# sqliteai/sqlite-vector

Measured on AMD Instinct MI355X. Metric: vectors scanned/sec, L2 top-20 over Nx384 f32, higher is better.
Workload: dtype f32; 1 GPU; 10Mx384 f32 L2 top-20 single-query; rows_per_gpu=10000000, dim=384, k=20, backend=HIP gfx950 x1

## Files before the change

### sqlite-vector_amd/csrc/vg_api.hip

```cpp
#include "vg_internal.h"

#include "vg_scan.h"


typedef void (*scan_fn_t)(ScanArgs);
scan_fn_t vg_pick_scan_kernel_ex(int vtype, int acc, int U);

typedef VgShape Shape;

static const int kAllowedU[] = {1, 2, 3, 4, 6, 8};

static int max_chunks_per_lane(int vtype, int acc, bool bf16_l2_u3) {
    if (vtype == VG_TYPE_F16) return 6;
    if (vtype == VG_TYPE_BF16) return (acc == A_L2 && !bf16_l2_u3) ? 6 : 3;
    return 8;
}

struct ShapeEnv { bool f16_round3, pref_round1, bf16_l2_u3, int_short_round3, force_long; int lpr_log2, u; };
static ShapeEnv shape_env() {
    ShapeEnv e;
    e.f16_round3 = vg_sw(SW_VG_SHAPE_F16_ROUND3, 0) != 0;
    e.pref_round1 = vg_sw(SW_VG_SHAPE_PREF_ROUND1, 0) != 0;
    e.bf16_l2_u3 = vg_sw(SW_VG_SHAPE_BF16_L2_U3, 0) != 0;
    e.int_short_round3 = vg_sw(SW_VG_SHAPE_INT_SHORT_ROUND3, 0) != 0;
// ... 143 lines not shown
        case VG_DIST_COSINE: return A_COS;
        case VG_DIST_DOT: return A_DOT;
        case VG_DIST_L1: return A_L1;
    }
    return -1;
}

static const char *type_tag(int t) {
    switch (t) { case VG_TYPE_F32: return "f32"; case VG_TYPE_F16: return "f16"; case VG_TYPE_BF16: return "bf16";
                 case VG_TYPE_U8: return "u8"; case VG_TYPE_I8: return "i8"; }
    return "?";
}
static const char *acc_tag(int a) {
    switch (a) { case A_L2: return "l2"; case A_COS: return "cos"; case A_DOT: return "dot"; case A_L1: return "l1"; case A_COSN: return "cosn"; }
    return "?";
}


extern "C" const char *vg_scan_kernel_name(vg_corpus *c, int metric) {
    if (!c) return "";
    Shape s;
    int acc = vg_metric_to_acc(metric);
    if (acc < 0 || !choose_shape(c->nch, c->vtype, acc, &s)) return "";
    if (acc == A_COS && (c->vtype == VG_TYPE_F16 || c->vtype == VG_TYPE_BF16) && !s.long_rows && vg_sw(SW_VG_HALF_COSN, 1)) acc = A_COSN;
    if (!s.long_rows && vg_scan_filter_name(c, metric, c->kernel_name, sizeof(c->kernel_name))) return c->kernel_name;
    snprintf(c->kernel_name, sizeof(c->kernel_name), "scan%s_%s_%s_u%d_lpr%d%s", s.long_rows ? "_long" : "",
             type_tag(c->vtype), acc_tag(acc), s.U, 1 << s.lpr_log2, use_nt_loads(c, c->n_rows) ? "_nt" : "");
    return c->kernel_name;
}



#define VG_MERGE_THREADS 1024
__global__ __launch_bounds__(VG_MERGE_THREADS) void vg_merge_kernel(const uint64_t *cand, int nlists, int k,
                                                                    uint64_t *out_keys, const unsigned long long *mirror_src,
                                                                    unsigned long long *mirror_dst) {
    __shared__ __attribute__((aligned(16))) uint8_t scratch[VG_SEL_SCRATCH_BYTES];
    if (mirror_dst && blockIdx.x == 0 && threadIdx.x < 3) mirror_dst[threadIdx.x] = mirror_src[threadIdx.x];
    vg_select_lists(cand + (long long)blockIdx.x * nlists * VG_WAVE, nlists, k, out_keys + (long long)blockIdx.x * VG_WAVE, scratch);
}

int vg_launch_merge(const uint64_t *dev_cand, int nlists, int k, uint64_t *dev_out_keys, int nq, hipStream_t stream) {
    hipLaunchKernelGGL(vg_merge_kernel, dim3((unsigned)nq), dim3(VG_MERGE_THREADS), 0, stream, dev_cand, nlists, k, dev_out_keys,
                       (const unsigned long long *)nullptr, (unsigned long long *)nullptr);
    return (int)hipGetLastError();
}

static int launch_scan(vg_corpus *c, int metric, const uint8_t *dev_query, int k, uint64_t *dev_out_keys,
                       float *dev_out_dist, hipStream_t stream, const ScanPlan &plan = ScanPlan());

int vg_launch_plain_scan(vg_corpus *c, int metric, const uint8_t *dev_query, int k, uint64_t *dev_out_keys, hipStream_t stream,
                         const ScanPlan &plan) {
    return launch_scan(c, metric, dev_query, k, dev_out_keys, nullptr, stream, plan);
}
int vg_launch_merge_one(const uint64_t *dev_cand, int nlists, int k, uint64_t *dev_out_keys, hipStream_t stream,
                        const unsigned long long *mirror_src, unsigned long long *mirror_dst) {
    hipLaunchKernelGGL(vg_merge_kernel, dim3(1), dim3(VG_MERGE_THREADS), 0, stream, dev_cand, nlists, k, dev_out_keys, mirror_src, mirror_dst);
    return (int)hipGetLastError();
}
int vg_plain_scan_shape(const vg_corpus *c, int metric, VgShape *out) {
    choose_shape(c->nch, c->vtype, vg_metric_to_acc(metric), out);
    return 0;
}
long long vg_plain_scan_blocks(const vg_corpus *c, int64_t n_rows, const VgShape &s) {
    const int rpb = VG_WAVE >> s.lpr_log2;
    const long long nbatch = (n_rows + rpb - 1) / rpb;
    const int bpc = std::max(1, std::min(8, vg_sw(SW_VG_BLOCKS_PER_CU, 1)));
    long long blocks = (nbatch + VG_WAVES_PER_BLOCK - 1) / VG_WAVES_PER_BLOCK;
    blocks = std::max<long long>(1, std::min<long long>(blocks, (long long)c->cu_count * bpc));
    blocks = std::min<long long>(blocks, VG_SEL_MAX_HEADS);
    blocks = std::min<long long>(blocks, std::max<long long>(32, nbatch / (2 * VG_WAVES_PER_BLOCK)));
    return blocks;
}

static int launch_scan(vg_corpus *c, int metric, const uint8_t *dev_query, int k, uint64_t *dev_out_keys,
                       float *dev_out_dist, hipStream_t stream, const ScanPlan &plan) {
    int acc = vg_metric_to_acc(metric);
    if (acc < 0) return vg_fail(VG_ERR_INVALID, "unknown distance metric %d", metric);
    const int64_t n_rows = (plan.n_rows >= 0) ? std::min<int64_t>(plan.n_rows, c->n_rows) : c->n_rows;
    if (plan.ref_emit) c->ref_prefix_rows = -1;
    Shape s;
    choose_shape(c->nch, c->vtype, acc, &s);
    const bool whole_prefix = plan.ref_emit && !dev_out_dist && plan.n_rows < 0 && k > 0 && k <= VG_MAX_FUSED_K && !s.long_rows &&
                              n_rows < VG_REF_EMIT_MIN_ROWS;
    if (!whole_prefix && plan.allow_filter && plan.n_rows < 0 && !dev_out_dist && k <= VG_MAX_FUSED_K) {
        int rcf = vg_launch_scan_filter(c, metric, dev_query, k, dev_out_keys, stream, plan.ref_emit, plan.final_out);
        if (rcf != -1) return rcf;
    }
    if (acc == A_COS && (c->vtype == VG_TYPE_F16 || c->vtype == VG_TYPE_BF16) && !s.long_rows && vg_sw(SW_VG_HALF_COSN, 1)) {
        int rcn = vg_ensure_row_norms(c);
        if (rcn != VG_OK) return rcn;
        acc = A_COSN;
        if (stream != c->stream) {
            if (!c->norm_ev) HIP_TRY(hipEventCreateWithFlags(&c->norm_ev, hipEventDisableTiming));
            HIP_TRY(hipEventRecord(c->norm_ev, c->stream));
            HIP_TRY(hipStreamWaitEvent(stream, c->norm_ev, 0));
        }
    }
    const bool emitting = plan.ref_emit && !dev_out_dist && !s.long_rows && plan.n_rows < 0 && k <= VG_MAX_FUSED_K &&
                          n_rows >= VG_REF_EMIT_MIN_ROWS;
    float *store_prefix = plan.store_prefix;
    unsigned long long *emit_reset = plan.emit_reset;
    if (whole_prefix) {
        int rcb = vg_ensure_ref_buffers(c, n_rows);
        if (rcb != VG_OK) return rcb;
        store_prefix = c->d_ref_prefix;
        emit_reset = c->d_below;
        c->ref_prefix_rows = n_rows;
    }
    const bool prefix_pass = store_prefix && !dev_out_dist && !s.long_rows && k > 0;
    scan_fn_t fn = (emitting || prefix_pass) ? vg_pick_scan_kernel_ex(c->vtype, acc, s.U) : pick_kernel(c->vtype, acc, s, use_nt_loads(c, n_rows));
    if (!fn) return vg_fail(VG_ERR_UNSUPPORTED, "no scan kernel for type %s", type_tag(c->vtype));

    const long long blocks = vg_plain_scan_blocks(c, n_rows, s);

    ScanArgs a{};
    a.rows = c->d_rows;
    a.query = dev_query;
    a.cand = plan.lists_out ? plan.lists_out : c->d_cand;
    a.out_dist = dev_out_dist;
    a.n_rows = n_rows;
    a.stride = c->stride;
    a.nch = c->nch;
    a.lpr_log2 = s.lpr_log2;
    a.k = k;
    a.root = (metric == VG_DIST_L2) ? 1 : 0;
    a.dim = c->dim;
    a.row_nn = (acc == A_COSN) ? c->d_xnorm : nullptr;
    a.init_keys = nullptr;
    a.emit = nullptr;
    a.emit_cap = 0;
    a.emit_reset = emit_reset;
    a.order = scan_order_for(c, n_rows);
    if (prefix_pass) a.out_dist = store_prefix;
    else a.emit_reset = nullptr;
    size_t qbytes = (size_t)c->nch * 16;
    if (s.long_rows) {
        const size_t slice = (size_t)VG_WAVE * VG_LONG_U;
        qbytes = ((c->nch + slice - 1) / slice) * slice * 16;
    }
    size_t smem = std::max<size_t>(qbytes, (size_t)VG_PUBLISH_LDS_BYTES);
    a.store_lds_off = 0;
    if (dev_out_dist && !s.long_rows) {
        a.store_lds_off = (int)((qbytes + 255) / 256 * 256);
        smem = std::max<size_t>(smem, (size_t)a.store_lds_off + (size_t)VG_WAVES_PER_BLOCK * VG_STORE_FLOATS * sizeof(float));
    }

    if (c->append_pending && stream != c->stream) HIP_TRY(hipStreamWaitEvent(stream, c->append_ev, 0));

    hipEvent_t *evs = plan.record ? vg_prof_slot(c, (uint8_t)((dev_out_dist == nullptr ? VG_EVF_MERGE : 0) | (emitting ? VG_EVF_PREPASS : 0))) : nullptr;
    if (evs) hipEventRecord(evs[0], stream);
    if (emitting) {
        const int64_t P = vg_ref_prefix_for(n_rows);
        int rcb = vg_ensure_ref_buffers(c, P);
        if (rcb != VG_OK) return rcb;
        ScanPlan pre;
        pre.n_rows = P;
        pre.allow_filter = false;
        pre.record = false;
        pre.store_prefix = c->d_ref_prefix;
        pre.emit_reset = c->d_below;
        int rcp = launch_scan(c, metric, dev_query, k, dev_out_keys, nullptr, stream, pre);
        if (rcp != VG_OK) return rcp;
        a.init_keys = dev_out_keys;
        a.emit = c->d_below;
        a.emit_cap = VG_BELOW_CAP;
        c->ref_prefix_rows = P;
        if (evs) hipEventRecord(evs[1], stream);
    }
    if (smem > 64 * 1024)
        HIP_TRY(hipFuncSetAttribute(reinterpret_cast<const void *>(fn), hipFuncAttributeMaxDynamicSharedMemorySize, (int)smem));
    hipLaunchKernelGGL(fn, dim3((unsigned)blocks), dim3(VG_BLOCK), smem, stream, a);
    if (evs) hipEventRecord(evs[2], stream);
    if (plan.lists_out) {
        if (plan.n_lists_out) *plan.n_lists_out = (int)blocks;
    } else if (!dev_out_dist) {
        hipLaunchKernelGGL(vg_merge_kernel, dim3(1), dim3(VG_MERGE_THREADS), 0, stream,
                           (const uint64_t *)c->d_cand, (int)blocks, k, plan.final_out ? plan.final_out : dev_out_keys,
                           (const unsigned long long *)nullptr, (unsigned long long *)nullptr);
    }
    if (evs) hipEventRecord(evs[3], stream);
    HIP_TRY(hipGetLastError());
    return VG_OK;
}

static bool host_direct(const vg_corpus *c) {
    const int v = vg_sw(SW_VG_HOST_DIRECT, -1);
    if (v >= 0) return v != 0;
    return c->n_rows * c->stride <= (64ll << 20);
}

static void stage_query(vg_corpus *c, const void *query) {
    memset(c->h_query, 0, (size_t)c->stride);
    memcpy(c->h_query, query, (size_t)c->dim * c->es);
}

static void slot_times(vg_corpus *c, int slot, float *scan_ms, float *merge_ms, float *prepass_ms) {
    hipEvent_t *evs = &c->ev[(size_t)slot * VG_PROF_EVS];
    const uint8_t fl = c->ev_flags[(size_t)slot];
    hipEventSynchronize(evs[3]);
    *scan_ms = 0.f; *merge_ms = 0.f; *prepass_ms = 0.f;
    if (fl & VG_EVF_PREPASS) hipEventElapsedTime(prepass_ms, evs[0], evs[1]);
    hipEventElapsedTime(scan_ms, evs[(fl & VG_EVF_PREPASS) ? 1 : 0], evs[2]);
    if (fl & VG_EVF_MERGE) hipEventElapsedTime(merge_ms, evs[2], evs[3]);
}

void vg_collect_timing(vg_corpus *c) {
    if (!c->profiling || c->prof_launches == 0) return;
    slot_times(c, (int)((c->prof_launches - 1) % VG_PROF_RING), &c->last_scan_ms, &c->last_merge_ms, &c->last_prepass_ms);
}

extern "C" float vg_key_distance(uint64_t key) { return vg_sortable_f32((uint32_t)(key >> 32)); }
extern "C" uint32_t vg_key_position(uint64_t key) { return (uint32_t)(key & 0xFFFFFFFFull); }

extern "C" int vg_scan_topk_device(vg_corpus *c, int metric, const void *dev_query, int k, uint64_t *dev_out_keys,
                                   void *stream) {
    if (!c || !dev_query || !dev_out_keys) return vg_fail(VG_ERR_INVALID, "vg_scan_topk_device: NULL argument");
    if (k < 1 || k > VG_MAX_FUSED_K) return vg_fail(VG_ERR_UNSUPPORTED, "vg_scan_topk_device: k must be in 1..%d", VG_MAX_FUSED_K);
    HIP_TRY(hipSetDevice(c->device));
    hipStream_t st = stream ? (hipStream_t)stream : c->stream;
    if (c->n_rows == 0) {
        HIP_TRY(hipMemsetAsync(dev_out_keys, 0xFF, VG_WAVE * sizeof(uint64_t), st));
        return VG_OK;
    }
    return launch_scan(c, metric, (const uint8_t *)dev_query, k, dev_out_keys, nullptr, st);
}

extern "C" int vg_scan_distances_device(vg_corpus *c, int metric, const void *dev_query, float *dev_out_dist, void *stream) {
    if (!c || !dev_query || !dev_out_dist) return vg_fail(VG_ERR_INVALID, "vg_scan_distances_device: NULL argument");
    HIP_TRY(hipSetDevice(c->device));
    if (c->n_rows == 0) return VG_OK;
    return launch_scan(c, metric, (const uint8_t *)dev_query, 0, nullptr, dev_out_dist, stream ? (hipStream_t)stream : c->stream);
}
// ... 279 lines not shown
```

### sqlite-vector_amd/csrc/vg_corpus.hip

```cpp
#include "vg_internal.h"

#include <atomic>
#include <mutex>
#include <utility>
#include <vector>

#include "vg_device.h"


static thread_local std::string g_err;

int vg_fail(int code, const char *fmt, ...) {
    char buf[1024];
    va_list ap;
    va_start(ap, fmt);
    vsnprintf(buf, sizeof(buf), fmt, ap);
    va_end(ap);
    g_err = buf;
    return code;
}

extern "C" const char *vg_last_error(void) { return g_err.c_str(); }
extern "C" void vg_set_last_error_(const char *msg) { g_err = msg ? msg : ""; }

// ... 16 lines not shown
        char arch[64];
        snprintf(arch, sizeof(arch), "%s", p.gcnArchName);
        char *colon = strchr(arch, ':');
        if (colon) *colon = 0;
        snprintf(name, sizeof(name), "HIP %s x%d", arch, n);
    } else {
        snprintf(name, sizeof(name), "HIP");
    }
    return name;
}


struct VgSwitchName { const char *name; int lab; };
static const VgSwitchName vg_switch_names[VGSW_COUNT] = {
    {"VECTORGPU_SHARD_GATHER", 0},
    {"VECTORGPU_SHARD_THREADS", 0},
    {"VG_BATCH_BPC", 1},
    {"VG_BATCH_H_SPLIT", 0},
    {"VG_BATCH_H_WAVES", 0},
    {"VG_BATCH_LONG", 0},
    {"VG_BATCH_LONG_BPC", 1},
    {"VG_BATCH_MFMA", 0},
    {"VG_BATCH_MIN_QUERIES", 1},
    {"VG_BATCH_PREPASS", 1},
    {"VG_BATCH_Q8", 0},
    {"VG_BATCH_SLICE", 0},
    {"VG_BATCH_STAGES", 0},
    {"VG_BATCH_TILE_MAJOR", 0},
    {"VG_BLOCKS_PER_CU", 1},
    {"VG_F32_FILTER", 0},
    {"VG_FILTER_LPR_LOG2", 1},
    {"VG_FILTER_U", 1},
    {"VG_FORCE_LONG", 0},
    {"VG_HALF_COSN", 1},
    {"VG_HOST_DIRECT", 1},
    {"VG_KEYS_DIRECT", 1},
    {"VG_LPR_LOG2", 1},
    {"VG_MULTI_SCAN", 0},
    {"VG_NT", 1},
    {"VG_Q8_TWO_READS", 1},
    {"VG_RADIX_SELECT", 0},
    {"VG_REF_ALWAYS_EMIT", 1},
    {"VG_REF_STORE_MODE", 0},
    {"VG_SCAN_FILTER", 0},
    {"VG_SCAN_FILTER_MIN_MB", 0},
    {"VG_SCAN_FILTER_MIRROR_COPY", 1},
    {"VG_SCAN_FILTER_N4", 0},
    {"VG_SCAN_FILTER_NO_GUARD", 0},
    {"VG_SCAN_FILTER_PREMERGE", 1},
    {"VG_SCAN_FILTER_PREPASS", 1},
    {"VG_SCAN_FILTER_PREPASS_DIV", 1},
    {"VG_SCAN_FILTER_SHADOW", 0},
    {"VG_SCAN_ORDER", 1},
    {"VG_SHAPE_BF16_L2_U3", 1},
    {"VG_SHAPE_F16_ROUND3", 1},
    {"VG_SHAPE_INT_SHORT_ROUND3", 1},
    {"VG_SHAPE_PREF_ROUND1", 1},
    {"VG_U", 1},
};
std::atomic<int> vg_switch_values[VGSW_COUNT];
void vg_switches_read(void) {
    for (int i = 0; i < VGSW_COUNT; ++i) {
        int v = VGSW_UNSET;
#ifndef VG_LAB
        if (!vg_switch_names[i].lab)
#endif
// ... 9 lines not shown
    }
}
__attribute__((constructor)) static void vg_switches_at_load(void) { vg_switches_read(); }
extern "C" void vg_reload_switches(void) { vg_switches_read(); }

extern "C" int vg_corpus_create(int device, int vtype, int dim, int64_t capacity_rows_hint, vg_corpus **out) {
    if (!out) return vg_fail(VG_ERR_INVALID, "vg_corpus_create: out is NULL");
    *out = nullptr;
    vg_switches_read();
    int es = vg_elem_size(vtype);
    if (es == 0) return vg_fail(VG_ERR_INVALID, "vg_corpus_create: unknown vector type %d", vtype);
    if (dim <= 0) return vg_fail(VG_ERR_INVALID, "vg_corpus_create: dimension must be positive (got %d)", dim);
    int ndev = vg_device_count();
    if (ndev <= 0) return vg_fail(VG_ERR_NO_DEVICE, "no HIP device available (the scan path is GPU-only)");
    if (device < 0 || device >= ndev) return vg_fail(VG_ERR_INVALID, "device %d out of range (0..%d)", device, ndev - 1);
    int64_t row_bytes = (int64_t)dim * es;
    if (row_bytes > 128 * 1024) return vg_fail(VG_ERR_UNSUPPORTED, "rows larger than 128 KiB are not supported (dim=%d): the query must fit the CU's 160 KiB LDS", dim);
    HIP_TRY(hipSetDevice(device));
    vg_corpus *c = new vg_corpus();
    c->device = device;
    c->vtype = vtype;
    c->dim = dim;
    c->es = es;
    c->nch = (int)((row_bytes + 15) / 16);
    c->stride = (int64_t)c->nch * 16;
    hipDeviceProp_t p;
    if (hipGetDeviceProperties(&p, device) != hipSuccess) { delete c; return vg_fail(VG_ERR_HIP, "hipGetDeviceProperties failed"); }
    c->cu_count = p.multiProcessorCount;
    c->max_blocks = c->cu_count * 8;
    hipError_t e;
    if ((e = hipStreamCreateWithFlags(&c->stream, hipStreamNonBlocking)) != hipSuccess ||
        (e = hipMalloc(&c->d_query, (size_t)c->stride)) != hipSuccess ||
        (e = hipHostMalloc(&c->h_query, (size_t)c->stride)) != hipSuccess ||
        (e = hipMalloc(&c->d_cand, (size_t)c->max_blocks * VG_WAVE * sizeof(uint64_t))) != hipSuccess ||
        (e = hipMalloc(&c->d_keys, VG_WAVE * sizeof(uint64_t))) != hipSuccess ||
        (e = hipHostMalloc(&c->h_keys, VG_WAVE * sizeof(uint64_t))) != hipSuccess) {
        vg_corpus_destroy(c);
        return vg_fail(VG_ERR_HIP, "vg_corpus_create: device setup failed: %s", hipGetErrorString(e));
    }
    if (capacity_rows_hint > 0) {
        e = hipMalloc(&c->d_rows, (size_t)(capacity_rows_hint * c->stride));
        if (e != hipSuccess) {
            vg_corpus_destroy(c);
            return vg_fail(VG_ERR_NOMEM, "vg_corpus_create: cannot allocate %lld bytes of HBM: %s",
                           (long long)(capacity_rows_hint * c->stride), hipGetErrorString(e));
        }
        c->cap_rows = capacity_rows_hint;
    }
    *out = c;
    return VG_OK;
}

extern "C" void vg_corpus_destroy(vg_corpus *c) {
    if (!c) return;
    hipSetDevice(c->device);
    if (c->stream) hipStreamSynchronize(c->stream);
    if (c->d_rows) hipFree(c->d_rows);
    if (c->d_query) hipFree(c->d_query);
    if (c->h_query) hipHostFree(c->h_query);
    if (c->d_cand) hipFree(c->d_cand);
    if (c->d_cand_pre) hipFree(c->d_cand_pre);
    if (c->d_keys) hipFree(c->d_keys);
    if (c->h_keys) hipHostFree(c->h_keys);
    if (c->d_dist) hipFree(c->d_dist);
    if (c->d_sel_keys) hipFree(c->d_sel_keys);
    if (c->d_sel_sorted) hipFree(c->d_sel_sorted);
    if (c->d_sel_temp) hipFree(c->d_sel_temp);
    for (int i = 0; i < 2; ++i) { if (c->pin[i]) hipHostFree(c->pin[i]); if (c->pin_ev[i]) hipEventDestroy(c->pin_ev[i]); }
    if (c->append_ev) hipEventDestroy(c->append_ev);
    if (c->d_stage) hipFree(c->d_stage);
    if (c->d_bq) hipFree(c->d_bq);
    if (c->h_bq) hipHostFree(c->h_bq);
// ... 677 lines not shown
```

### sqlite-vector_amd/csrc/vg_device.h

```cpp
#pragma once

#include <hip/hip_runtime.h>
#include <stdint.h>

#define VG_EMPTY_KEY 0xFFFFFFFFFFFFFFFFull
#define VG_WAVE 64
#define VG_BLOCK 1024
#define VG_WAVES_PER_BLOCK (VG_BLOCK / VG_WAVE)
#define VG_MAX_FUSED_K 64

enum { T_F32 = 1, T_F16 = 2, T_BF16 = 3, T_U8 = 4, T_I8 = 5 };
enum { M_L2 = 1, M_SQL2 = 2, M_COS = 3, M_DOT = 4, M_L1 = 5 };
enum { A_L2 = 0, A_COS = 1, A_DOT = 2, A_L1 = 3, A_COSN = 4  };

struct ScanArgs {
    const uint8_t *rows;
    const uint8_t *query;
    uint64_t *cand;
    float *out_dist;
    long long n_rows;
    long long stride;
    int nch;
    int lpr_log2;
    int k;
    int root;
    int dim;
    const float *row_nn;
    int store_lds_off;
    const uint64_t *init_keys;
    unsigned long long *emit;
    unsigned emit_cap;
    unsigned long long *emit_reset;
    int order;
    float within_r;
    unsigned long long within_cap;
    const uint64_t *mask;
};


__host__ __device__ inline uint32_t vg_f32_sortable(float d) {
    uint32_t b;
#if defined(__HIP_DEVICE_COMPILE__)
    b = __float_as_uint(d);
#else
    __builtin_memcpy(&b, &d, 4);
#endif
    return b ^ ((b >> 31) ? 0xFFFFFFFFu : 0x80000000u);
}
__host__ __device__ inline float vg_sortable_f32(uint32_t s) {
    uint32_t b = s ^ ((s >> 31) ? 0x80000000u : 0xFFFFFFFFu);
#if defined(__HIP_DEVICE_COMPILE__)
    return __uint_as_float(b);
#else
    float f; __builtin_memcpy(&f, &b, 4); return f;
#endif
}
__host__ __device__ inline uint64_t vg_make_key(float d, uint32_t pos) {
    return ((uint64_t)vg_f32_sortable(d) << 32) | (uint64_t)pos;
}


__device__ inline uint64_t vg_readlane64(uint64_t v, int lane_uniform) {
    uint32_t lo = (uint32_t)__builtin_amdgcn_readlane((int)(uint32_t)v, lane_uniform);
    uint32_t hi = (uint32_t)__builtin_amdgcn_readlane((int)(uint32_t)(v >> 32), lane_uniform);
    return ((uint64_t)hi << 32) | lo;
}

__device__ inline uint64_t vg_wave_shr1(uint64_t v) {
    const uint32_t lo = (uint32_t)__builtin_amdgcn_update_dpp(0, (int)(uint32_t)v, 0x138, 0xf, 0xf, false);
// ... 112 lines not shown
```

### sqlite-vector_amd/csrc/vg_internal.h

```cpp
#pragma once

#include "../../include/vectorgpu.h"
#include "../../include/vectorgpu_diag.h"

#include <hip/hip_runtime.h>

#include <algorithm>
#include <cmath>
#include <cstdarg>
#include <cstdio>
#include <cstdlib>
#include <cstring>
#include <string>
#include <vector>

#define VG_PROF_RING 1024
#define VG_PROF_EVS 4
#define VG_EVF_MERGE 1
#define VG_EVF_PREPASS 2
#define VG_WAVE_HOST 64

int vg_fail(int code, const char *fmt, ...);

#define HIP_TRY(expr)                                                                                     \
    do {                                                                                                  \
        hipError_t e__ = (expr);                                                                          \
        if (e__ != hipSuccess)                                                                            \
            return vg_fail(e__ == hipErrorOutOfMemory ? VG_ERR_NOMEM : VG_ERR_HIP, "%s failed: %s (%s:%d)", \
                           #expr, hipGetErrorString(e__), __FILE__, __LINE__);                            \
    } while (0)


static inline int vg_elem_size(int vtype) {
    switch (vtype) {
        case VG_TYPE_F32: return 4;
        case VG_TYPE_F16: case VG_TYPE_BF16: return 2;
        case VG_TYPE_U8: case VG_TYPE_I8: return 1;
    }
    return 0;
}

struct vg_corpus {
    int device = 0;
    int vtype = 0;
    int dim = 0;
    int es = 0;
    int nch = 0;
    int64_t stride = 0;
    int64_t n_rows = 0;
    int64_t cap_rows = 0;
    uint8_t *d_rows = nullptr;
    std::vector<int64_t> rowids;
    bool rowids_ascending = true;
    int64_t rowid_base = 1;

    hipStream_t stream = nullptr;
    uint8_t *d_query = nullptr;
    uint8_t *h_query = nullptr;
    uint64_t *d_cand = nullptr;
    uint64_t *d_cand_pre = nullptr;
    uint64_t *d_keys = nullptr;
    uint64_t *h_keys = nullptr;
    float *d_dist = nullptr;
    int64_t d_dist_cap = 0;
    int64_t dist_valid_rows = 0;
    unsigned long long *d_below = nullptr;
    uint8_t *h_ref = nullptr;
    size_t h_ref_bytes = 0;
    std::vector<uint64_t> ref_pairs;
    int tie_order = 0;
    float *d_ref_prefix = nullptr;
    int64_t ref_prefix_cap = 0;
    int64_t ref_prefix_rows = -1;
    int ref_hot = 0;
    unsigned long long ref_stats[4] = {0, 0, 0, 0};
    uint64_t *d_sel_keys = nullptr, *d_sel_sorted = nullptr;
    void *d_sel_temp = nullptr;
    uint32_t *d_sel_state = nullptr;
    size_t sel_temp_bytes = 0;
    int64_t sel_cap = 0;
    uint8_t *pin[2] = {nullptr, nullptr};
    hipEvent_t pin_ev[2] = {nullptr, nullptr};
    bool pin_busy[2] = {false, false};
    int pin_idx = 0;
    uint8_t *d_stage = nullptr;
    hipEvent_t append_ev = nullptr;
    bool append_pending = false;
    bool enqueued = false;
    float *d_xnorm = nullptr;
    int64_t xnorm_rows = 0, xnorm_cap = 0;
    hipEvent_t norm_ev = nullptr;
    uint32_t *d_sx = nullptr;
// ... 96 lines not shown
    if (p > VG_REF_PREFIX_MAX) p = VG_REF_PREFIX_MAX;
    return p;
}
int vg_ensure_ref_buffers(vg_corpus *c, int64_t prefix_rows);
#define VG_REF_FIRST_PAIRS 8191
int vg_ref_emitted_enqueue(vg_corpus *c);
int vg_ref_emitted_wait(vg_corpus *c, const float **prefix, int64_t *prefix_rows, unsigned long long **pairs, unsigned long long *count,
                        bool *overflow);
struct VgRefSlots;
void vg_ref_offer_run(VgRefSlots &slots, const float *d, int64_t n, int64_t g0);
int vg_ref_replay_slab(vg_corpus *c, int metric, const void *query, int k, VgRefSlots &slots, int64_t gbase, bool fresh);

static inline void vg_drop_mask(vg_corpus *c) { c->mask_count = -1; c->mask_host.clear(); }
int vg_mask_upload(vg_corpus *c);

static inline hipEvent_t *vg_prof_slot(vg_corpus *c, uint8_t flags) {
    if (!c->profiling) return nullptr;
    const int slot = (int)(c->prof_launches % VG_PROF_RING);
    c->ev_flags[(size_t)slot] = flags;
    ++c->prof_launches;
    return &c->ev[(size_t)slot * VG_PROF_EVS];
}

int vg_metric_to_acc(int metric);
void vg_collect_timing(vg_corpus *c);
int vg_ensure_row_norms(vg_corpus *c);
struct VgShape { int lpr_log2; int U; bool long_rows; };
bool vg_choose_shape(int nch, int vtype, int acc, VgShape *out, int u_cap);
int vg_launch_merge(const uint64_t *dev_cand, int nlists, int k, uint64_t *dev_out_keys, int nq, hipStream_t stream);
int vg_launch_plain_scan(vg_corpus *c, int metric, const uint8_t *dev_query, int k, uint64_t *dev_out_keys, hipStream_t stream,
                         const ScanPlan &plan);
int vg_launch_merge_one(const uint64_t *dev_cand, int nlists, int k, uint64_t *dev_out_keys, hipStream_t stream,
                        const unsigned long long *mirror_src = nullptr, unsigned long long *mirror_dst = nullptr);
int vg_plain_scan_shape(const vg_corpus *c, int metric, VgShape *out);
long long vg_plain_scan_blocks(const vg_corpus *c, int64_t n_rows, const VgShape &s);
int vg_launch_scan_filter(vg_corpus *c, int metric, const uint8_t *dev_query, int k, uint64_t *dev_out_keys, hipStream_t stream,
                          bool ref_emit = false, uint64_t *final_out = nullptr);
int vg_scan_topk_enqueue_plan(vg_corpus *c, int metric, const void *query, int k, bool ref_emit);
bool vg_scan_filter_would_serve(const vg_corpus *c, int metric, int k);
bool vg_scan_filter_policy(const vg_corpus *c);
int vg_ensure_filter_counters(vg_corpus *c);
bool vg_scan_filter_name(vg_corpus *c, int metric, char *out, size_t out_len);
bool vg_batch_keys_are_scan_exact(const vg_corpus *c, int metric, int k);
long long vg_bf16_shadow_stride(const vg_corpus *c);
int vg_ensure_bf16_shadow(vg_corpus *c);
int vg_ensure_q8_shadow(vg_corpus *c);
int vg_multi_queries_per_pass(const vg_corpus *c, int metric);
int vg_launch_scan_multi(vg_corpus *c, int metric, const uint8_t *dev_queries, int k, uint64_t *dev_cand,
                         uint64_t *dev_out_keys, hipStream_t stream);
int vg_multi_plan(const vg_corpus *c, int metric, VgShape *s);
```

### sqlite-vector_amd/csrc/vg_scan.h

```cpp
#pragma once

#include "vg_accum.h"
#include "vg_lists.h"

#define VG_PUBLISH_LDS_BYTES (VG_WAVES_PER_BLOCK * VG_WAVE * 8 + VG_SEL_SCRATCH_BYTES)

__device__ inline void vg_block_publish(uint8_t *smem, uint64_t mine, int k, uint64_t *dst) {
    const int lane = threadIdx.x & (VG_WAVE - 1);
    const int wave = threadIdx.x >> 6;
    uint64_t *lists = reinterpret_cast<uint64_t *>(smem);
    lists[wave * VG_WAVE + lane] = (lane < k) ? mine : VG_EMPTY_KEY;
    __syncthreads();
    vg_select_lists(lists, VG_WAVES_PER_BLOCK, k, dst, smem + VG_WAVES_PER_BLOCK * VG_WAVE * 8);
}

typedef uint32_t vg_u32x4 __attribute__((ext_vector_type(4)));

template <bool NT>
__device__ inline uint4 vg_load16(const uint8_t *p) {
    if (NT) {
        vg_u32x4 v = __builtin_nontemporal_load(reinterpret_cast<const vg_u32x4 *>(p));
        return make_uint4(v.x, v.y, v.z, v.w);
    }
    return *reinterpret_cast<const uint4 *>(p);
}

#ifndef VG_LOAD_PREDICATED
#define VG_LOAD_PREDICATED 0
#endif
static __device__ __attribute__((aligned(16))) uint32_t vg_zero_chunk[4] = {0u, 0u, 0u, 0u};

template <int U, bool NT>
__device__ inline void vg_load_batch(uint4 (&dst)[U], const uint8_t *rows, long long row, long long n_rows,
                                     long long stride, int sub, int lpr, int nch) {
    const uint8_t *p = rows + row * stride + (long long)sub * 16;
#pragma unroll
    for (int u = 0; u < U; ++u) {
        const int c = sub + u * lpr;
        if (VG_LOAD_PREDICATED) {
            uint4 v = make_uint4(0u, 0u, 0u, 0u);
            if (row < n_rows && c < nch) v = vg_load16<NT>(p + (long long)u * lpr * 16);
            dst[u] = v;
        } else {
            const uint8_t *src = (row < n_rows && c < nch) ? p + (long long)u * lpr * 16 : reinterpret_cast<const uint8_t *>(vg_zero_chunk);
            dst[u] = vg_load16<NT>(src);
        }
// ... 27 lines not shown
    queued += __popcll(m);
    if (queued > VG_WITHIN_QUEUE - VG_WAVE) vg_within_flush(queue, queued, out, cap, lane);
}

__device__ inline uint64_t vg_mask_bits(const uint64_t *mask, long long row0, int n, bool in_range) {
    const uint32_t r = (uint32_t)__builtin_amdgcn_readfirstlane((int)(in_range ? (uint32_t)row0 : 0xFFFFFFFFu));
    const bool ok = r != 0xFFFFFFFFu;
    const uint64_t bits = mask[ok ? (r >> 6) : 0u] >> (r & 63u);
    const uint64_t keep = (n >= VG_WAVE) ? ~0ull : ((1ull << (n & 63)) - 1ull);
    return ok ? (bits & keep) : 0ull;
}

template <int VT, int ACC, int U, bool NT, bool EX = false, bool WITHIN = false, bool MASKED = false>
__global__ __launch_bounds__(VG_BLOCK) void vg_scan_kernel(ScanArgs a) {
    extern __shared__ __attribute__((aligned(16))) uint8_t smem[];
    __shared__ VgListExtras ex;
    const int lane = threadIdx.x & (VG_WAVE - 1);
    const int wave = threadIdx.x >> 6;
    const int lpr_log2 = a.lpr_log2;
    const int lpr = 1 << lpr_log2;
    const int rpb = VG_WAVE >> lpr_log2;
    const int sub = lane & (lpr - 1);
    const int rib = lane >> lpr_log2;

    uint4 *qs = reinterpret_cast<uint4 *>(smem);
    for (int c = threadIdx.x; c < a.nch; c += VG_BLOCK) qs[c] = reinterpret_cast<const uint4 *>(a.query)[c];
    const int k = a.k;
    uint64_t mine = VG_EMPTY_KEY;
    uint64_t thr = VG_EMPTY_KEY;
    if constexpr (EX) {
        if (k > 0) thr = vg_list_extras_init(&ex, a.init_keys, k, a.emit, a.emit_cap);
        if (a.emit_reset && blockIdx.x == 0 && threadIdx.x == 0) *a.emit_reset = 0ull;
    }
    __syncthreads();
    uint4 q[U];
#pragma unroll
    for (int u = 0; u < U; ++u) {
        const int c = sub + u * lpr;
        q[u] = (c < a.nch) ? qs[c] : make_uint4(0u, 0u, 0u, 0u);
    }
    const typename Accum<VT, ACC>::QStat qstat = Accum<VT, ACC>::template query_stat<U>(q, lpr_log2);
    const bool store_mode = (WITHIN || MASKED) ? false : EX ? ((a.out_dist != nullptr) && k == 0) : (a.out_dist != nullptr);
    const bool store_too = EX && (a.out_dist != nullptr) && k != 0;

    const long long nbatch = (a.n_rows + rpb - 1) / rpb;
    const long long nwaves = (long long)gridDim.x * VG_WAVES_PER_BLOCK;
    const long long gw = (long long)blockIdx.x * VG_WAVES_PER_BLOCK + wave;
    const int flush_every = VG_STORE_FLOATS / rpb;
    long long per_wave = (nbatch + nwaves - 1) / nwaves;
    per_wave = ((per_wave + flush_every - 1) / flush_every) * flush_every;
    long long wstride = store_mode ? 1 : nwaves;
    long long b = store_mode ? gw * per_wave : gw;
    long long b_end = store_mode ? ((gw + 1) * per_wave < nbatch ? (gw + 1) * per_wave : nbatch) : nbatch;
    if (a.order == 1 && !store_mode) {
        const long long per_block = (nbatch + gridDim.x - 1) / gridDim.x;
        wstride = VG_WAVES_PER_BLOCK;
        b = (long long)blockIdx.x * per_block + wave;
        b_end = ((long long)blockIdx.x + 1) * per_block < nbatch ? ((long long)blockIdx.x + 1) * per_block : nbatch;
    }
    float *line = reinterpret_cast<float *>(smem + a.store_lds_off) + wave * VG_STORE_FLOATS;
    int in_line = 0;
    long long line_row0 = b * rpb;
    uint64_t *wqueue = reinterpret_cast<uint64_t *>(smem + a.store_lds_off) + wave * VG_WITHIN_QUEUE;
    int wqueued = 0;
#ifndef VG_RING_F32
#define VG_RING_F32 0
// ... 94 lines not shown
#pragma unroll
        for (int j = 0; j < NB - 1; ++j) load(buf[j], nn[j], b + j * wstride);
        while (b < b_end) {
#pragma unroll
            for (int j = 0; j < NB; ++j) {
                const long long bj = b + j * wstride;
                load(buf[(j + NB - 1) % NB], nn[(j + NB - 1) % NB], bj + (NB - 1) * wstride);
                if (bj < b_end) process(buf[j], nn[j], bj);
            }
            b += NB * wstride;
        }
    } else {
        load(buf[0], nn[0], b);
        while (b < b_end) {
            const long long bn = b + wstride;
            load(buf[1], nn[1], bn);
            process(buf[0], nn[0], b);
#pragma unroll
            for (int u = 0; u < U; ++u) buf[0][u] = buf[1][u];
            nn[0] = nn[1];
            b = bn;
        }
    }
    if constexpr (WITHIN) {
        if (wqueued > 0) vg_within_flush(wqueue, wqueued, a.emit, a.within_cap, lane);
        return;
    }
    if (store_mode) {
        for (int j = lane; j < in_line * rpb && line_row0 + j < a.n_rows; j += VG_WAVE) a.out_dist[line_row0 + j] = line[j];
        return;
    }

    __syncthreads();
    vg_block_publish(smem, mine, k, a.cand + (long long)blockIdx.x * VG_WAVE);
}

#define VG_LONG_U 2
template <int VT, int ACC, bool NT, bool WITHIN = false, bool MASKED = false>
__global__ __launch_bounds__(VG_BLOCK) void vg_scan_long_kernel(ScanArgs a) {
    extern __shared__ __attribute__((aligned(16))) uint8_t smem[];
    const int lane = threadIdx.x & (VG_WAVE - 1);
    const int wave = threadIdx.x >> 6;
    constexpr int U = VG_LONG_U;
    const int slice = VG_WAVE * U;
    const int S = (a.nch + slice - 1) / slice;
    const int nch_pad = S * slice;

    uint4 *qs = reinterpret_cast<uint4 *>(smem);
    for (int c = threadIdx.x; c < nch_pad; c += VG_BLOCK)
        qs[c] = (c < a.nch) ? reinterpret_cast<const uint4 *>(a.query)[c] : make_uint4(0u, 0u, 0u, 0u);
    __syncthreads();

    typename Accum<VT, ACC>::QStat qstat;
    {
        uint4 q0[U];
#pragma unroll
        for (int u = 0; u < U; ++u) q0[u] = qs[u * VG_WAVE + lane];
        qstat = Accum<VT, ACC>::template query_stat<U>(q0, 6);
        for (int s = 1; s < S; ++s) {
#pragma unroll
            for (int u = 0; u < U; ++u) q0[u] = qs[s * slice + u * VG_WAVE + lane];
            Accum<VT, ACC>::merge_qstat(qstat, Accum<VT, ACC>::template query_stat<U>(q0, 6));
        }
    }

    uint64_t mine = VG_EMPTY_KEY, thr = VG_EMPTY_KEY;
    const int k = a.k;
    const bool store_mode = (WITHIN || MASKED) ? false : (a.out_dist != nullptr);
    uint64_t *wqueue = reinterpret_cast<uint64_t *>(smem + a.store_lds_off) + wave * VG_WITHIN_QUEUE;
    int wqueued = 0;
    const long long wstride = (long long)gridDim.x * VG_WAVES_PER_BLOCK;
    const long long gw = (long long)blockIdx.x * VG_WAVES_PER_BLOCK + wave;

    auto load_slice = [&](uint4 (&dst)[U], long long row, int s, bool live = true) {
#pragma unroll
        for (int u = 0; u < U; ++u) {
            const int c = s * slice + u * VG_WAVE + lane;
            if (VG_LOAD_PREDICATED) {
                uint4 v = make_uint4(0u, 0u, 0u, 0u);
                if (row < a.n_rows && live && c < a.nch) v = vg_load16<NT>(a.rows + row * a.stride + (long long)c * 16);
                dst[u] = v;
            } else {
                dst[u] = vg_load16<NT>((row < a.n_rows && live && c < a.nch) ? a.rows + row * a.stride + (long long)c * 16
// ... 24 lines not shown
        }
        if (ns == 0 && (!MASKED || m_cur)) {
            float d = acc.finish(qstat, 6, a.root);
            if constexpr (VT == T_F16 || VT == T_BF16) {
                if (acc.special(qstat, 6) && lane == 0)
                    d = vg_slow_distance<VT, ACC>(reinterpret_cast<const uint16_t *>(qs),
                                                  reinterpret_cast<const uint16_t *>(a.rows + row * a.stride), a.dim, a.root);
            }
            d = vg_clamp(d);
            if constexpr (WITHIN) {
                vg_within_offer(vg_make_key(d, (uint32_t)row), (lane == 0) && (d <= a.within_r) && (d < INFINITY), wqueue, wqueued, a.emit, a.within_cap, lane);
            } else if (store_mode) {
                if (lane == 0) a.out_dist[row] = d;
            } else {
                vg_list_offer(vg_make_key(d, (uint32_t)row), (lane == 0) && (d < INFINITY), mine, thr, lane, k);
            }
            acc.init();
        }
        if constexpr (MASKED) {
            if (ns == 0) { m_cur = m_nxt; m_nxt = vg_mask_bits(a.mask, nrow + wstride, 1, nrow + wstride < a.n_rows) != 0ull; }
        }
#pragma unroll
        for (int u = 0; u < U; ++u) cur[u] = nxt[u];
        row = nrow;
        s = ns;
    }
    if constexpr (WITHIN) {
        if (wqueued > 0) vg_within_flush(wqueue, wqueued, a.emit, a.within_cap, lane);
        return;
    }
    if (store_mode) return;

    __syncthreads();
    vg_block_publish(smem, mine, k, a.cand + (long long)blockIdx.x * VG_WAVE);
}


template <int VT>
__global__ __launch_bounds__(256) void vg_half_rownorm_kernel(const uint8_t *rows, long long row0, long long n, long long stride,
                                                              int nch, float *out) {
    const int sub = threadIdx.x & 15;
    const long long group = ((long long)blockIdx.x * blockDim.x + threadIdx.x) >> 4;
    const long long ngroups = ((long long)gridDim.x * blockDim.x) >> 4;
    for (long long r = group; r < n; r += ngroups) {
        const uint4 *p = reinterpret_cast<const uint4 *>(rows + (row0 + r) * stride);
        double s0 = 0.0, s1 = 0.0, s2 = 0.0, s3 = 0.0;
        for (int c = sub; c < nch; c += 16) {
            const uint4 v = p[c];
            const uint32_t w[4] = {v.x, v.y, v.z, v.w};
#pragma unroll
            for (int j = 0; j < 4; ++j) {
                float lo, hi;
                vg_unpack2<VT>(w[j], lo, hi);
                if (j & 1) { s2 += (double)(lo * lo); s3 += (double)(hi * hi); }
                else { s0 += (double)(lo * lo); s1 += (double)(hi * hi); }
            }
        }
        const double s = vg_group_sum((s0 + s1) + (s2 + s3), 4);
        if (sub == 0) { const float f = (float)s; out[row0 + r] = (s > 0.0 && f == 0.0f) ? 1.401298464324817e-45f : f; }
    }
}
```

### sqlite-vector_amd/csrc/vg_scan_masked.hip

```cpp
#include "vg_internal.h"

#include "vg_scan.h"

typedef void (*scan_fn_t)(ScanArgs);

template <int VT, int ACC>
static scan_fn_t pick_u(int U) {
    switch (U) {
        case 1: return vg_scan_kernel<VT, ACC, 1, true, false, false, true>;
        case 2: return vg_scan_kernel<VT, ACC, 2, true, false, false, true>;
        case 3: return vg_scan_kernel<VT, ACC, 3, true, false, false, true>;
        case 4: return vg_scan_kernel<VT, ACC, 4, true, false, false, true>;
        case 6: return vg_scan_kernel<VT, ACC, 6, true, false, false, true>;
        case 8: return vg_scan_kernel<VT, ACC, 8, true, false, false, true>;
    }
    return nullptr;
}

template <int VT>
static scan_fn_t pick_acc(int acc, int U, bool long_rows) {
    if (long_rows) {
        switch (acc) {
            case A_L2: return vg_scan_long_kernel<VT, A_L2, true, false, true>;
            case A_COS: return vg_scan_long_kernel<VT, A_COS, true, false, true>;
// ... 83 lines not shown
    return VG_OK;
}

extern "C" int64_t vg_corpus_mask_count(const vg_corpus *c) { return c ? c->mask_count : -1; }


static int launch_masked(vg_corpus *c, int metric, int k) {
    int acc = vg_metric_to_acc(metric);
    VgShape s;
    vg_plain_scan_shape(c, metric, &s);
    if (acc == A_COS && (c->vtype == VG_TYPE_F16 || c->vtype == VG_TYPE_BF16) && !s.long_rows && vg_sw(SW_VG_HALF_COSN, 1)) {
        int rcn = vg_ensure_row_norms(c);
        if (rcn != VG_OK) return rcn;
        acc = A_COSN;
    }
    scan_fn_t fn = pick_masked_kernel(c->vtype, acc, s);
    if (!fn) return vg_fail(VG_ERR_UNSUPPORTED, "vg_scan_topk_masked: no kernel for this type / metric");

    const long long blocks = vg_plain_scan_blocks(c, c->n_rows, s);

    ScanArgs a{};
    a.rows = c->d_rows;
    a.query = c->d_query;
    a.cand = c->d_cand;
    a.n_rows = c->n_rows;
    a.stride = c->stride;
    a.nch = c->nch;
    a.lpr_log2 = s.lpr_log2;
    a.k = k;
    a.root = (metric == VG_DIST_L2) ? 1 : 0;
    a.dim = c->dim;
    a.row_nn = (acc == A_COSN) ? c->d_xnorm : nullptr;
    a.mask = c->d_mask;
    size_t qbytes = (size_t)c->nch * 16;
    if (s.long_rows) {
        const size_t slice = (size_t)VG_WAVE * VG_LONG_U;
        qbytes = ((c->nch + slice - 1) / slice) * slice * 16;
    }
    const size_t smem = std::max<size_t>(qbytes, (size_t)VG_PUBLISH_LDS_BYTES);

    hipEvent_t *evs = vg_prof_slot(c, VG_EVF_MERGE);
    if (evs) hipEventRecord(evs[0], c->stream);
    if (smem > 64 * 1024)
        HIP_TRY(hipFuncSetAttribute(reinterpret_cast<const void *>(fn), hipFuncAttributeMaxDynamicSharedMemorySize, (int)smem));
    hipLaunchKernelGGL(fn, dim3((unsigned)blocks), dim3(VG_BLOCK), smem, c->stream, a);
    if (evs) hipEventRecord(evs[2], c->stream);
    int rcm = vg_launch_merge_one(c->d_cand, (int)blocks, k, c->d_keys, c->stream);
    if (evs) hipEventRecord(evs[3], c->stream);
    if (rcm != 0) return vg_fail(VG_ERR_HIP, "vg_scan_topk_masked: merge launch failed: %s", hipGetErrorString((hipError_t)rcm));
    HIP_TRY(hipGetLastError());
    HIP_TRY(hipMemcpyAsync(c->h_keys, c->d_keys, VG_WAVE * sizeof(uint64_t), hipMemcpyDeviceToHost, c->stream));
    HIP_TRY(hipStreamSynchronize(c->stream));
    return VG_OK;
}

extern "C" int vg_scan_topk_masked_keys(vg_corpus *c, int metric, const void *query, int k, uint64_t *out_keys, int *out_count) {
    if (!c || !query || !out_count) return vg_fail(VG_ERR_INVALID, "vg_scan_topk_masked: NULL argument");
    *out_count = 0;
    if (k < 1) return vg_fail(VG_ERR_INVALID, "vg_scan_topk_masked: k must be at least 1");
    if (k > VG_MAX_FUSED_K) return vg_fail(VG_ERR_UNSUPPORTED, "vg_scan_topk_masked: k must be in 1..%d (masked scans use the fused list only)", VG_MAX_FUSED_K);
    if (!out_keys) return vg_fail(VG_ERR_INVALID, "vg_scan_topk_masked: NULL output");
    if (vg_metric_to_acc(metric) < 0) return vg_fail(VG_ERR_INVALID, "unknown distance metric %d", metric);
    if (c->mask_count < 0) return vg_fail(VG_ERR_INVALID, "vg_scan_topk_masked: no row mask set");
    if (c->mask_count == 0 || c->n_rows == 0) return VG_OK;
    HIP_TRY(hipSetDevice(c->device));
    c->enqueued = false;
    memset(c->h_query, 0, (size_t)c->stride);
    memcpy(c->h_query, query, (size_t)c->dim * c->es);
    HIP_TRY(hipMemcpyAsync(c->d_query, c->h_query, (size_t)c->stride, hipMemcpyHostToDevice, c->stream));
    int rc = launch_masked(c, metric, k);
    if (rc != VG_OK) return rc;
    vg_collect_timing(c);
    int cnt = 0;
    while (cnt < k && c->h_keys[cnt] != VG_EMPTY_KEY) { out_keys[cnt] = c->h_keys[cnt]; ++cnt; }
    *out_count = cnt;
    return VG_OK;
}

extern "C" int vg_scan_topk_masked(vg_corpus *c, int metric, const void *query, int k, int64_t *out_rowids, double *out_dist,
                                   int *out_count) {
    if (!c || !query || !out_count) return vg_fail(VG_ERR_INVALID, "vg_scan_topk_masked: NULL argument");
    *out_count = 0;
// ... 13 lines not shown
```

### sqlite-vector_amd/csrc/vg_switches.h

```cpp
#pragma once
#include <atomic>
#include <climits>

enum VgSwitch {
    SW_VECTORGPU_SHARD_GATHER,
    SW_VECTORGPU_SHARD_THREADS,
    SW_VG_BATCH_BPC,
    SW_VG_BATCH_H_SPLIT,
    SW_VG_BATCH_H_WAVES,
    SW_VG_BATCH_LONG,
    SW_VG_BATCH_LONG_BPC,
    SW_VG_BATCH_MFMA,
    SW_VG_BATCH_MIN_QUERIES,
    SW_VG_BATCH_PREPASS,
    SW_VG_BATCH_Q8,
    SW_VG_BATCH_SLICE,
    SW_VG_BATCH_STAGES,
    SW_VG_BATCH_TILE_MAJOR,
    SW_VG_BLOCKS_PER_CU,
    SW_VG_F32_FILTER,
    SW_VG_FILTER_LPR_LOG2,
    SW_VG_FILTER_U,
    SW_VG_FORCE_LONG,
    SW_VG_HALF_COSN,
    SW_VG_HOST_DIRECT,
    SW_VG_KEYS_DIRECT,
    SW_VG_LPR_LOG2,
    SW_VG_MULTI_SCAN,
    SW_VG_NT,
    SW_VG_Q8_TWO_READS,
    SW_VG_RADIX_SELECT,
    SW_VG_REF_ALWAYS_EMIT,
    SW_VG_REF_STORE_MODE,
    SW_VG_SCAN_FILTER,
    SW_VG_SCAN_FILTER_MIN_MB,
    SW_VG_SCAN_FILTER_MIRROR_COPY,
    SW_VG_SCAN_FILTER_N4,
    SW_VG_SCAN_FILTER_NO_GUARD,
    SW_VG_SCAN_FILTER_PREMERGE,
    SW_VG_SCAN_FILTER_PREPASS,
    SW_VG_SCAN_FILTER_PREPASS_DIV,
    SW_VG_SCAN_FILTER_SHADOW,
    SW_VG_SCAN_ORDER,
    SW_VG_SHAPE_BF16_L2_U3,
    SW_VG_SHAPE_F16_ROUND3,
    SW_VG_SHAPE_INT_SHORT_ROUND3,
    SW_VG_SHAPE_PREF_ROUND1,
    SW_VG_U,
    VGSW_COUNT
};
#define VGSW_UNSET INT_MIN
extern std::atomic<int> vg_switch_values[VGSW_COUNT];
void vg_switches_read(void);
static inline int vg_sw(VgSwitch id, int dflt) { const int v = vg_switch_values[id].load(std::memory_order_relaxed); return v == VGSW_UNSET ? dflt : v; }
static inline bool vg_sw_set(VgSwitch id) { return vg_switch_values[id].load(std::memory_order_relaxed) != VGSW_UNSET; }
```

Before: 4.452 billion vectors/s.

## Fuse final top-k merge into scan kernel via last-block-arrives select

```diff
diff --git a/sqlite-vector_amd/csrc/vg_api.hip b/sqlite-vector_amd/csrc/vg_api.hip
--- a/sqlite-vector_amd/csrc/vg_api.hip
+++ b/sqlite-vector_amd/csrc/vg_api.hip
@@ -199,6 +199,7 @@
 
 
 #define VG_MERGE_THREADS 1024
+static_assert(VG_MERGE_THREADS == VG_BLOCK, "the fused select must run vg_select_lists with the merge kernel's thread count");
 __global__ __launch_bounds__(VG_MERGE_THREADS) void vg_merge_kernel(const uint64_t *cand, int nlists, int k,
                                                                     uint64_t *out_keys, const unsigned long long *mirror_src,
                                                                     unsigned long long *mirror_dst) {
@@ -215,6 +216,7 @@
 
 static int launch_scan(vg_corpus *c, int metric, const uint8_t *dev_query, int k, uint64_t *dev_out_keys,
                        float *dev_out_dist, hipStream_t stream, const ScanPlan &plan = ScanPlan());
+bool vg_fused_select(void) { return vg_sw(SW_VG_FUSED_SELECT, 1) != 0; }
 
 int vg_launch_plain_scan(vg_corpus *c, int metric, const uint8_t *dev_query, int k, uint64_t *dev_out_keys, hipStream_t stream,
                          const ScanPlan &plan) {
@@ -280,11 +282,15 @@
     if (!fn) return vg_fail(VG_ERR_UNSUPPORTED, "no scan kernel for type %s", type_tag(c->vtype));
 
     const long long blocks = vg_plain_scan_blocks(c, n_rows, s);
+    const bool fused = vg_fused_select() && !dev_out_dist && !plan.lists_out && !emitting && !prefix_pass &&
+                       (s.long_rows || vg_fused_tail_shape(c->vtype, acc, s.U));
 
     ScanArgs a{};
     a.rows = c->d_rows;
     a.query = dev_query;
     a.cand = plan.lists_out ? plan.lists_out : c->d_cand;
+    a.arrive = fused ? c->d_arrive : nullptr;
+    a.fin_out = fused ? (plan.final_out ? plan.final_out : dev_out_keys) : nullptr;
     a.out_dist = dev_out_dist;
     a.n_rows = n_rows;
     a.stride = c->stride;
@@ -306,7 +312,7 @@
         const size_t slice = (size_t)VG_WAVE * VG_LONG_U;
         qbytes = ((c->nch + slice - 1) / slice) * slice * 16;
     }
-    size_t smem = std::max<size_t>(qbytes, (size_t)VG_PUBLISH_LDS_BYTES);
+    size_t smem = (emitting || prefix_pass) ? std::max<size_t>(qbytes, (size_t)VG_PUBLISH_LDS_BYTES) : vg_fused_lds_bytes(qbytes);
     a.store_lds_off = 0;
     if (dev_out_dist && !s.long_rows) {
         a.store_lds_off = (int)((qbytes + 255) / 256 * 256);
@@ -315,7 +321,7 @@
 
     if (c->append_pending && stream != c->stream) HIP_TRY(hipStreamWaitEvent(stream, c->append_ev, 0));
 
-    hipEvent_t *evs = plan.record ? vg_prof_slot(c, (uint8_t)((dev_out_dist == nullptr ? VG_EVF_MERGE : 0) | (emitting ? VG_EVF_PREPASS : 0))) : nullptr;
+    hipEvent_t *evs = plan.record ? vg_prof_slot(c, (uint8_t)(fused ? VG_EVF_FUSED : ((dev_out_dist == nullptr ? VG_EVF_MERGE : 0) | (emitting ? VG_EVF_PREPASS : 0)))) : nullptr;
     if (evs) hipEventRecord(evs[0], stream);
     if (emitting) {
         const int64_t P = vg_ref_prefix_for(n_rows);
@@ -339,6 +345,10 @@
         HIP_TRY(hipFuncSetAttribute(reinterpret_cast<const void *>(fn), hipFuncAttributeMaxDynamicSharedMemorySize, (int)smem));
     hipLaunchKernelGGL(fn, dim3((unsigned)blocks), dim3(VG_BLOCK), smem, stream, a);
     if (evs) hipEventRecord(evs[2], stream);
+    if (fused) {
+        HIP_TRY(hipGetLastError());
+        return VG_OK;
+    }
     if (plan.lists_out) {
         if (plan.n_lists_out) *plan.n_lists_out = (int)blocks;
     } else if (!dev_out_dist) {
@@ -365,7 +375,7 @@
 static void slot_times(vg_corpus *c, int slot, float *scan_ms, float *merge_ms, float *prepass_ms) {
     hipEvent_t *evs = &c->ev[(size_t)slot * VG_PROF_EVS];
     const uint8_t fl = c->ev_flags[(size_t)slot];
-    hipEventSynchronize(evs[3]);
+    hipEventSynchronize(evs[(fl & VG_EVF_FUSED) ? 2 : 3]);
     *scan_ms = 0.f; *merge_ms = 0.f; *prepass_ms = 0.f;
     if (fl & VG_EVF_PREPASS) hipEventElapsedTime(prepass_ms, evs[0], evs[1]);
     hipEventElapsedTime(scan_ms, evs[(fl & VG_EVF_PREPASS) ? 1 : 0], evs[2]);
diff --git a/sqlite-vector_amd/csrc/vg_corpus.hip b/sqlite-vector_amd/csrc/vg_corpus.hip
--- a/sqlite-vector_amd/csrc/vg_corpus.hip
+++ b/sqlite-vector_amd/csrc/vg_corpus.hip
@@ -72,6 +72,7 @@
     {"VG_FILTER_LPR_LOG2", 1},
     {"VG_FILTER_U", 1},
     {"VG_FORCE_LONG", 0},
+    {"VG_FUSED_SELECT", 0},
     {"VG_HALF_COSN", 1},
     {"VG_HOST_DIRECT", 1},
     {"VG_KEYS_DIRECT", 1},
@@ -147,12 +148,15 @@
     if ((e = hipStreamCreateWithFlags(&c->stream, hipStreamNonBlocking)) != hipSuccess ||
         (e = hipMalloc(&c->d_query, (size_t)c->stride)) != hipSuccess ||
         (e = hipHostMalloc(&c->h_query, (size_t)c->stride)) != hipSuccess ||
-        (e = hipMalloc(&c->d_cand, (size_t)c->max_blocks * VG_WAVE * sizeof(uint64_t))) != hipSuccess ||
+        (e = hipMalloc(&c->d_cand, (size_t)c->max_blocks * VG_WAVE * sizeof(uint64_t) + VG_ARRIVE_BYTES)) != hipSuccess ||
+        (e = hipMemsetAsync(c->d_cand + (size_t)c->max_blocks * VG_WAVE, 0, VG_ARRIVE_BYTES, c->stream)) != hipSuccess ||
+        (e = hipStreamSynchronize(c->stream)) != hipSuccess ||
         (e = hipMalloc(&c->d_keys, VG_WAVE * sizeof(uint64_t))) != hipSuccess ||
         (e = hipHostMalloc(&c->h_keys, VG_WAVE * sizeof(uint64_t))) != hipSuccess) {
         vg_corpus_destroy(c);
         return vg_fail(VG_ERR_HIP, "vg_corpus_create: device setup failed: %s", hipGetErrorString(e));
     }
+    c->d_arrive = reinterpret_cast<unsigned int *>(c->d_cand + (size_t)c->max_blocks * VG_WAVE);
     if (capacity_rows_hint > 0) {
         e = hipMalloc(&c->d_rows, (size_t)(capacity_rows_hint * c->stride));
         if (e != hipSuccess) {
diff --git a/sqlite-vector_amd/csrc/vg_device.h b/sqlite-vector_amd/csrc/vg_device.h
--- a/sqlite-vector_amd/csrc/vg_device.h
+++ b/sqlite-vector_amd/csrc/vg_device.h
@@ -35,6 +35,8 @@
     float within_r;
     unsigned long long within_cap;
     const uint64_t *mask;
+    unsigned int *arrive;
+    uint64_t *fin_out;
 };
 
 
diff --git a/sqlite-vector_amd/csrc/vg_internal.h b/sqlite-vector_amd/csrc/vg_internal.h
--- a/sqlite-vector_amd/csrc/vg_internal.h
+++ b/sqlite-vector_amd/csrc/vg_internal.h
@@ -18,7 +18,9 @@
 #define VG_PROF_EVS 4
 #define VG_EVF_MERGE 1
 #define VG_EVF_PREPASS 2
+#define VG_EVF_FUSED 4
 #define VG_WAVE_HOST 64
+#define VG_ARRIVE_BYTES 128
 
 int vg_fail(int code, const char *fmt, ...);
 
@@ -58,6 +60,7 @@
     uint8_t *d_query = nullptr;
     uint8_t *h_query = nullptr;
     uint64_t *d_cand = nullptr;
+    unsigned int *d_arrive = nullptr;
     uint64_t *d_cand_pre = nullptr;
     uint64_t *d_keys = nullptr;
     uint64_t *h_keys = nullptr;
@@ -220,6 +223,7 @@
                          const ScanPlan &plan);
 int vg_launch_merge_one(const uint64_t *dev_cand, int nlists, int k, uint64_t *dev_out_keys, hipStream_t stream,
                         const unsigned long long *mirror_src = nullptr, unsigned long long *mirror_dst = nullptr);
+bool vg_fused_select(void);
 int vg_plain_scan_shape(const vg_corpus *c, int metric, VgShape *out);
 long long vg_plain_scan_blocks(const vg_corpus *c, int64_t n_rows, const VgShape &s);
 int vg_launch_scan_filter(vg_corpus *c, int metric, const uint8_t *dev_query, int k, uint64_t *dev_out_keys, hipStream_t stream,
diff --git a/sqlite-vector_amd/csrc/vg_scan.h b/sqlite-vector_amd/csrc/vg_scan.h
--- a/sqlite-vector_amd/csrc/vg_scan.h
+++ b/sqlite-vector_amd/csrc/vg_scan.h
@@ -12,6 +12,53 @@
     lists[wave * VG_WAVE + lane] = (lane < k) ? mine : VG_EMPTY_KEY;
     __syncthreads();
     vg_select_lists(lists, VG_WAVES_PER_BLOCK, k, dst, smem + VG_WAVES_PER_BLOCK * VG_WAVE * 8);
+}
+
+struct VgFusedTail {
+    uint64_t own[VG_WAVE];
+    uint64_t *cand;
+    uint64_t *fin_out;
+    unsigned int *arrive;
+    unsigned int nblocks;
+    unsigned int last;
+};
+__host__ __device__ constexpr bool vg_fused_tail_shape(int vt, int acc, int U) {
+    return !((vt == T_F16 && U > 6) || (vt == T_BF16 && U > (acc == A_L2 ? 6 : 3)));
+}
+__host__ __device__ inline size_t vg_fused_tail_off(size_t qbytes) { return qbytes > (size_t)VG_PUBLISH_LDS_BYTES ? qbytes : (size_t)VG_PUBLISH_LDS_BYTES; }
+__host__ __device__ inline size_t vg_fused_lds_bytes(size_t qbytes) { return vg_fused_tail_off(qbytes) + sizeof(VgFusedTail); }
+__device__ inline void vg_fused_tail_init(VgFusedTail *ft) {
+    if (threadIdx.x == 0) {
+        const __attribute__((address_space(4))) ScanArgs *ka = (const __attribute__((address_space(4))) ScanArgs *)__builtin_amdgcn_kernarg_segment_ptr();
+        ft->cand = ka->cand; ft->fin_out = ka->fin_out; ft->arrive = ka->arrive; ft->nblocks = gridDim.x;
+    }
+}
+
+__device__ inline void vg_block_publish_select(uint8_t *smem, VgFusedTail *ft, uint64_t mine, int k) {
+    const int lane = threadIdx.x & (VG_WAVE - 1);
+    const int wave = threadIdx.x >> 6;
+    uint64_t *lists = reinterpret_cast<uint64_t *>(smem);
+    uint8_t *scratch = smem + VG_WAVES_PER_BLOCK * VG_WAVE * 8;
+    uint64_t *cand = ft->cand;
+    uint64_t *fin_out = ft->fin_out;
+    lists[wave * VG_WAVE + lane] = (lane < k) ? mine : VG_EMPTY_KEY;
+    __syncthreads();
+    if (!fin_out) {
+        vg_select_lists(lists, VG_WAVES_PER_BLOCK, k, cand + (long long)blockIdx.x * VG_WAVE, scratch);
+        return;
+    }
+    vg_select_lists(lists, VG_WAVES_PER_BLOCK, k, ft->own, scratch);
+    __syncthreads();
+    if (wave == 0) {
+        cand[(long long)blockIdx.x * VG_WAVE + lane] = ft->own[lane];
+        __threadfence();
+        if (lane == 0) ft->last = (atomicAdd(ft->arrive, 1u) == ft->nblocks - 1u) ? 1u : 0u;
+    }
+    __syncthreads();
+    if (ft->last == 0u) return;
+    __threadfence();
+    vg_select_lists(cand, (int)ft->nblocks, k, fin_out, scratch);
+    if (threadIdx.x == 0) __hip_atomic_store(ft->arrive, 0u, __ATOMIC_RELAXED, __HIP_MEMORY_SCOPE_AGENT);
 }
 
 typedef uint32_t vg_u32x4 __attribute__((ext_vector_type(4)));
@@ -105,6 +152,8 @@
         if (k > 0) thr = vg_list_extras_init(&ex, a.init_keys, k, a.emit, a.emit_cap);
         if (a.emit_reset && blockIdx.x == 0 && threadIdx.x == 0) *a.emit_reset = 0ull;
     }
+    constexpr bool FUSE = !EX && !WITHIN && vg_fused_tail_shape(VT, ACC, U);
+    if constexpr (FUSE) vg_fused_tail_init(reinterpret_cast<VgFusedTail *>(smem + vg_fused_tail_off(0)));
     __syncthreads();
     uint4 q[U];
 #pragma unroll
@@ -265,7 +314,8 @@
     }
 
     __syncthreads();
-    vg_block_publish(smem, mine, k, a.cand + (long long)blockIdx.x * VG_WAVE);
+    if constexpr (FUSE) vg_block_publish_select(smem, reinterpret_cast<VgFusedTail *>(smem + vg_fused_tail_off(0)), mine, k);
+    else vg_block_publish(smem, mine, k, a.cand + (long long)blockIdx.x * VG_WAVE);
 }
 
 #define VG_LONG_U 2
@@ -282,6 +332,7 @@
     uint4 *qs = reinterpret_cast<uint4 *>(smem);
     for (int c = threadIdx.x; c < nch_pad; c += VG_BLOCK)
         qs[c] = (c < a.nch) ? reinterpret_cast<const uint4 *>(a.query)[c] : make_uint4(0u, 0u, 0u, 0u);
+    if constexpr (!WITHIN) vg_fused_tail_init(reinterpret_cast<VgFusedTail *>(smem + vg_fused_tail_off((size_t)nch_pad * 16)));
     __syncthreads();
 
     typename Accum<VT, ACC>::QStat qstat;
@@ -372,7 +423,8 @@
     if (store_mode) return;
 
     __syncthreads();
-    vg_block_publish(smem, mine, k, a.cand + (long long)blockIdx.x * VG_WAVE);
+    if constexpr (!WITHIN) vg_block_publish_select(smem, reinterpret_cast<VgFusedTail *>(smem + vg_fused_tail_off((size_t)S * slice * 16)), mine, k);
+    else vg_block_publish(smem, mine, k, a.cand + (long long)blockIdx.x * VG_WAVE);
 }
 
 
diff --git a/sqlite-vector_amd/csrc/vg_scan_masked.hip b/sqlite-vector_amd/csrc/vg_scan_masked.hip
--- a/sqlite-vector_amd/csrc/vg_scan_masked.hip
+++ b/sqlite-vector_amd/csrc/vg_scan_masked.hip
@@ -139,22 +139,27 @@
     a.dim = c->dim;
     a.row_nn = (acc == A_COSN) ? c->d_xnorm : nullptr;
     a.mask = c->d_mask;
+    const bool fused = vg_fused_select() && (s.long_rows || vg_fused_tail_shape(c->vtype, acc, s.U));
+    a.arrive = fused ? c->d_arrive : nullptr;
+    a.fin_out = fused ? c->d_keys : nullptr;
     size_t qbytes = (size_t)c->nch * 16;
     if (s.long_rows) {
         const size_t slice = (size_t)VG_WAVE * VG_LONG_U;
         qbytes = ((c->nch + slice - 1) / slice) * slice * 16;
     }
-    const size_t smem = std::max<size_t>(qbytes, (size_t)VG_PUBLISH_LDS_BYTES);
-
-    hipEvent_t *evs = vg_prof_slot(c, VG_EVF_MERGE);
+    const size_t smem = vg_fused_lds_bytes(qbytes);
+
+    hipEvent_t *evs = vg_prof_slot(c, fused ? VG_EVF_FUSED : VG_EVF_MERGE);
     if (evs) hipEventRecord(evs[0], c->stream);
     if (smem > 64 * 1024)
         HIP_TRY(hipFuncSetAttribute(reinterpret_cast<const void *>(fn), hipFuncAttributeMaxDynamicSharedMemorySize, (int)smem));
     hipLaunchKernelGGL(fn, dim3((unsigned)blocks), dim3(VG_BLOCK), smem, c->stream, a);
     if (evs) hipEventRecord(evs[2], c->stream);
-    int rcm = vg_launch_merge_one(c->d_cand, (int)blocks, k, c->d_keys, c->stream);
-    if (evs) hipEventRecord(evs[3], c->stream);
-    if (rcm != 0) return vg_fail(VG_ERR_HIP, "vg_scan_topk_masked: merge launch failed: %s", hipGetErrorString((hipError_t)rcm));
+    if (!fused) {
+        int rcm = vg_launch_merge_one(c->d_cand, (int)blocks, k, c->d_keys, c->stream);
+        if (evs) hipEventRecord(evs[3], c->stream);
+        if (rcm != 0) return vg_fail(VG_ERR_HIP, "vg_scan_topk_masked: merge launch failed: %s", hipGetErrorString((hipError_t)rcm));
+    }
     HIP_TRY(hipGetLastError());
     HIP_TRY(hipMemcpyAsync(c->h_keys, c->d_keys, VG_WAVE * sizeof(uint64_t), hipMemcpyDeviceToHost, c->stream));
     HIP_TRY(hipStreamSynchronize(c->stream));
diff --git a/sqlite-vector_amd/csrc/vg_switches.h b/sqlite-vector_amd/csrc/vg_switches.h
--- a/sqlite-vector_amd/csrc/vg_switches.h
+++ b/sqlite-vector_amd/csrc/vg_switches.h
@@ -22,6 +22,7 @@
     SW_VG_FILTER_LPR_LOG2,
     SW_VG_FILTER_U,
     SW_VG_FORCE_LONG,
+    SW_VG_FUSED_SELECT,
     SW_VG_HALF_COSN,
     SW_VG_HOST_DIRECT,
     SW_VG_KEYS_DIRECT,
```

Result: slower. 4.406 billion vectors/s (-1.0%).
